# yhao-wang/DenseRetrievalToolkits

Hardware: AMD Instinct MI355X
Metric: queries/sec@top-1000, 10Mx768 corpus (BASELINE: passages encoded/sec + queries/sec@top-1000, 10Mx768 corpus, 1/2/4/8 GPU) (higher is better)
Workload: dtype bf16

## Files before the change

### denseretrievaltoolkits_amd/csrc/select.hip

```cpp
#include "profile.h"
#include "search_internal.h"

namespace drt {

constexpr int kSelThreads = 512;
constexpr int kSelWaves = kSelThreads / 64;
constexpr int kSelBins = 1024;
constexpr int kSelBuf = 4096;
constexpr int kSelKPT = 16;
constexpr int kSelRegCap = kSelKPT * kSelThreads;

template <int INPUT>
__device__ __forceinline__ uint64_t sel_load(const SelectArgs& a, int64_t q, int64_t j) {
  if (INPUT == SEL_KEYS64) return ((const uint64_t*)a.in)[q * a.in_stride + j];
  const uint32_t v = ((const uint32_t*)a.in)[q * a.in_stride + j];
  return ((uint64_t)v << 32) | (uint64_t)(uint32_t)j;
}

__device__ __forceinline__ float key_score(uint64_t x) { return desc_key_to_score((uint32_t)(x >> 32)); }

__device__ __forceinline__ int score_bin(float s, float smin, float scale) {
  if (scale == 0.0f) return 0;
  return hist_bin((s - smin) * scale, kSelBins, __builtin_signbit(s) ? 0 : kSelBins - 1);
}
// ... 41 lines not shown
#pragma unroll
  for (int size = 2; size <= N; size <<= 1) {
#pragma unroll
    for (int stride = size >> 1; stride > 0; stride >>= 1) {
      if (stride >= NT) {
        if (E >= 2 && stride == NT) sort_inthread<T, NT, E, 1>(v, size, tid);
        else if (E >= 4 && stride == 2 * NT) sort_inthread<T, NT, E, 2>(v, size, tid);
        else if (E >= 8) sort_inthread<T, NT, E, 4>(v, size, tid);
      } else {
        T p[E];
        if (stride >= 64) {
#pragma unroll
          for (int u = 0; u < E; ++u) buf[u * NT + tid] = v[u];
          __syncthreads();
#pragma unroll
          for (int u = 0; u < E; ++u) p[u] = buf[(u * NT + tid) ^ stride];
          __syncthreads();
        } else {
#pragma unroll
          for (int u = 0; u < E; ++u) p[u] = __shfl_xor(v[u], stride, 64);
        }
#pragma unroll
        for (int u = 0; u < E; ++u) {
          const int i = u * NT + tid;
          const bool keep_min = ((i & stride) == 0) == ((i & size) == 0);
          const T a = v[u], b = p[u];
          v[u] = keep_min ? (a < b ? a : b) : (a < b ? b : a);
        }
      }
    }
  }
#pragma unroll
  for (int u = 0; u < E; ++u) {
    const int i = u * NT + tid;
    if (i < n) buf[i] = v[u];
  }
  __syncthreads();
}

template <typename T, int NT>
__device__ __forceinline__ void block_sort(T* buf, int n) {
  if (n <= 1) {
    __syncthreads();
    return;
  }
  if (n <= NT) block_sort_fixed<T, NT, NT>(buf, n);
  else if (n <= 2 * NT) block_sort_fixed<T, NT, 2 * NT>(buf, n);
  else if (n <= 4 * NT) block_sort_fixed<T, NT, 4 * NT>(buf, n);
  else block_sort_fixed<T, NT, 8 * NT>(buf, n);
}

__device__ __forceinline__ void block_bitonic(uint64_t* buf, int n2) { block_sort<uint64_t, kSelThreads>(buf, n2); }

template <int INPUT, int OUTPUT>
__global__ __launch_bounds__(kSelThreads) void select_kernel(SelectArgs a) {
  __shared__ uint32_t hist[kSelWaves][kSelBins];
  __shared__ uint32_t suffix[kSelBins];
  __shared__ float fscr[kSelWaves];
  __shared__ uint64_t uscr[kSelWaves];
  __shared__ uint64_t sh_prefix, sh_mask;
  __shared__ int64_t sh_kk;
  __shared__ int sh_done, sh_bin;
  __shared__ uint32_t sh_nsel, sh_nside;
  __shared__ __attribute__((aligned(16))) uint64_t buf[kSelBuf];

  const int tid = threadIdx.x;
  const int wave = tid >> 6;
  const int64_t q = blockIdx.x;
  int64_t c_raw, c;
  if (INPUT == SEL_KEYS64) {
    c_raw = a.counts[q * kCntStride];
    c = c_raw < a.cap ? c_raw : a.cap;
  } else {
    c_raw = a.n_in;
    c = a.n_in;
  }
  const int64_t kk_total = (int64_t)a.k < c ? (int64_t)a.k : c;

  if (OUTPUT == SEL_KTH && (c < (int64_t)a.k || c == 0)) {
    if (tid == 0) a.tau[q] = -__builtin_inff();
    return;
  }

  bool fast_done = false;
  int nsel = 0;
  if (c > (int64_t)a.k && c <= kSelRegCap) {
    uint64_t kr[kSelKPT];
    float sc[kSelKPT];
#pragma unroll
    for (int u = 0; u < kSelKPT; ++u) {
      const int64_t j = (int64_t)u * kSelThreads + tid;
      const uint64_t x = sel_load<INPUT>(a, q, j < c ? j : 0);
      kr[u] = j < c ? x : ~0ull;
    }
    float lo = __builtin_inff(), hi = -__builtin_inff();
#pragma unroll
    for (int u = 0; u < kSelKPT; ++u) {
      sc[u] = key_score(kr[u]);
      if ((int64_t)u * kSelThreads + tid < c) {
        lo = fminf(lo, sc[u]);
        hi = fmaxf(hi, sc[u]);
      }
    }
    lo = block_reduce(lo, fscr, [](float x, float y) { return fminf(x, y); });
    hi = block_reduce(hi, fscr, [](float x, float y) { return fmaxf(x, y); });
    const float range = hi - lo;
    const float scale = hist_scale((float)kSelBins, range);
    for (int i = tid; i < kSelWaves * kSelBins; i += kSelThreads) (&hist[0][0])[i] = 0;
    __syncthreads();
    int bn[kSelKPT];
#pragma unroll
    for (int u = 0; u < kSelKPT; ++u) {
      bn[u] = -1;
      if ((int64_t)u * kSelThreads + tid < c) {
        bn[u] = score_bin(sc[u], lo, scale);
        atomicAdd(&hist[wave][bn[u]], 1u);
      }
    }
    __syncthreads();
    for (int i = tid; i < kSelBins; i += kSelThreads) {
      uint32_t t = 0;
#pragma unroll
      for (int w = 0; w < kSelWaves; ++w) t += hist[w][i];
      suffix[i] = t;
    }
    __syncthreads();
    for (int off = 1; off < kSelBins; off <<= 1) {
      uint32_t v[kSelBins / kSelThreads];
#pragma unroll
      for (int u = 0; u < kSelBins / kSelThreads; ++u) {
        const int i = tid + u * kSelThreads;
        v[u] = suffix[i] + (i + off < kSelBins ? suffix[i + off] : 0u);
      }
      __syncthreads();
#pragma unroll
      for (int u = 0; u < kSelBins / kSelThreads; ++u) suffix[tid + u * kSelThreads] = v[u];
      __syncthreads();
    }
    if (tid == 0) sh_bin = 0;
    __syncthreads();
    for (int i = tid; i < kSelBins; i += kSelThreads) {
      const bool ok = (int64_t)suffix[i] >= kk_total;
      const bool next_ok = (i + 1 < kSelBins) && (int64_t)suffix[i + 1] >= kk_total;
      if (ok && !next_ok) sh_bin = i;
    }
    __syncthreads();
    const int b = sh_bin;
    if (OUTPUT == SEL_KTH) {
      float t = __builtin_inff();
#pragma unroll
      for (int u = 0; u < kSelKPT; ++u)
        if (bn[u] >= b) t = fminf(t, sc[u]);
      t = block_reduce(t, fscr, [](float x, float y) { return fminf(x, y); });
      if (tid == 0) a.tau[q] = t;
      return;
    }
    const uint32_t cnt_sel = suffix[b];
    const uint32_t c_above = (b + 1 < kSelBins) ? suffix[b + 1] : 0u;
    const uint32_t cnt_b = cnt_sel - c_above;
    if (cnt_b <= (uint32_t)(kSelBuf / 2) && kk_total <= kSelBuf / 2) {
      uint64_t* side = buf + kSelBuf / 2;
      if (tid == 0) {
        sh_nsel = 0;
        sh_nside = 0;
      }
      __syncthreads();
#pragma unroll
      for (int u = 0; u < kSelKPT; ++u) {
        if (bn[u] > b) buf[atomicAdd(&sh_nsel, 1u)] = kr[u];
        else if (bn[u] == b) side[atomicAdd(&sh_nside, 1u)] = kr[u];
      }
      __syncthreads();
      const int ns = (int)sh_nside;
      int m2 = 1;
      while (m2 < ns) m2 <<= 1;
      for (int i = ns + tid; i < m2; i += kSelThreads) side[i] = ~0ull;
      __syncthreads();
      block_bitonic(side, m2);
      const int need = (int)kk_total - (int)c_above;
      for (int i = tid; i < need; i += kSelThreads) buf[c_above + i] = side[i];
      __syncthreads();
      nsel = (int)kk_total;
      fast_done = true;
    } else if (cnt_sel <= (uint32_t)kSelBuf) {
      if (tid == 0) sh_nsel = 0;
      __syncthreads();
#pragma unroll
      for (int u = 0; u < kSelKPT; ++u)
        if (bn[u] >= b) buf[atomicAdd(&sh_nsel, 1u)] = kr[u];
      __syncthreads();
      nsel = (int)sh_nsel;
      fast_done = true;
    }
  } else if (c > (int64_t)a.k) {
    float lo = __builtin_inff(), hi = -__builtin_inff();
    for (int64_t j = tid; j < c; j += kSelThreads) {
      const float s = key_score(sel_load<INPUT>(a, q, j));
      lo = fminf(lo, s);
      hi = fmaxf(hi, s);
    }
    lo = block_reduce(lo, fscr, [](float x, float y) { return fminf(x, y); });
    hi = block_reduce(hi, fscr, [](float x, float y) { return fmaxf(x, y); });
    const float range = hi - lo;
    const float scale = hist_scale((float)kSelBins, range);
    for (int i = tid; i < kSelWaves * kSelBins; i += kSelThreads) (&hist[0][0])[i] = 0;
    __syncthreads();
    for (int64_t j = tid; j < c; j += kSelThreads) {
      const float s = key_score(sel_load<INPUT>(a, q, j));
      atomicAdd(&hist[wave][score_bin(s, lo, scale)], 1u);
    }
    __syncthreads();
    for (int i = tid; i < kSelBins; i += kSelThreads) {
      uint32_t t = 0;
#pragma unroll
      for (int w = 0; w < kSelWaves; ++w) t += hist[w][i];
      suffix[i] = t;
    }
    __syncthreads();
    for (int off = 1; off < kSelBins; off <<= 1) {
      uint32_t v[kSelBins / kSelThreads];
#pragma unroll
      for (int u = 0; u < kSelBins / kSelThreads; ++u) {
        const int i = tid + u * kSelThreads;
        v[u] = suffix[i] + (i + off < kSelBins ? suffix[i + off] : 0u);
      }
      __syncthreads();
#pragma unroll
      for (int u = 0; u < kSelBins / kSelThreads; ++u) suffix[tid + u * kSelThreads] = v[u];
      __syncthreads();
    }
    if (tid == 0) sh_bin = 0;
    __syncthreads();
    for (int i = tid; i < kSelBins; i += kSelThreads) {
      const bool ok = (int64_t)suffix[i] >= kk_total;
      const bool next_ok = (i + 1 < kSelBins) && (int64_t)suffix[i + 1] >= kk_total;
      if (ok && !next_ok) sh_bin = i;
    }
    __syncthreads();
    const int b = sh_bin;
    const uint32_t cnt_sel = suffix[b];
    if (OUTPUT == SEL_KTH) {
      float t = __builtin_inff();
      for (int64_t j = tid; j < c; j += kSelThreads) {
        const float s = key_score(sel_load<INPUT>(a, q, j));
        if (score_bin(s, lo, scale) >= b) t = fminf(t, s);
      }
      t = block_reduce(t, fscr, [](float x, float y) { return fminf(x, y); });
      if (tid == 0) a.tau[q] = t;
      return;
    }
    const uint32_t c_above = (b + 1 < kSelBins) ? suffix[b + 1] : 0u;
    const uint32_t cnt_b = cnt_sel - c_above;
    if (cnt_b <= (uint32_t)(kSelBuf / 2) && kk_total <= kSelBuf / 2) {
      uint64_t* side = buf + kSelBuf / 2;
      if (tid == 0) {
        sh_nsel = 0;
        sh_nside = 0;
      }
      __syncthreads();
      for (int64_t j = tid; j < c; j += kSelThreads) {
        const uint64_t x = sel_load<INPUT>(a, q, j);
        const int bx = score_bin(key_score(x), lo, scale);
        if (bx > b) buf[atomicAdd(&sh_nsel, 1u)] = x;
        else if (bx == b) side[atomicAdd(&sh_nside, 1u)] = x;
      }
      __syncthreads();
      const int ns = (int)sh_nside;
      int m2 = 1;
      while (m2 < ns) m2 <<= 1;
      for (int i = ns + tid; i < m2; i += kSelThreads) side[i] = ~0ull;
      __syncthreads();
      block_bitonic(side, m2);
      const int need = (int)kk_total - (int)c_above;
      for (int i = tid; i < need; i += kSelThreads) buf[c_above + i] = side[i];
      __syncthreads();
      nsel = (int)kk_total;
      fast_done = true;
    } else if (cnt_sel <= (uint32_t)kSelBuf) {
      if (tid == 0) sh_nsel = 0;
      __syncthreads();
      for (int64_t j = tid; j < c; j += kSelThreads) {
        const uint64_t x = sel_load<INPUT>(a, q, j);
        if (score_bin(key_score(x), lo, scale) >= b) {
          const uint32_t p = atomicAdd(&sh_nsel, 1u);
          if (p < (uint32_t)kSelBuf) buf[p] = x;
        }
      }
      __syncthreads();
      nsel = (int)sh_nsel;
      fast_done = true;
    }
  }

  if (!fast_done) {
    if (tid == 0) {
      sh_prefix = 0;
      sh_mask = 0;
      sh_kk = kk_total;
      sh_done = (c <= (int64_t)a.k) ? 1 : 0;
      if (c <= (int64_t)a.k) {
        sh_prefix = ~0ull;
        sh_mask = ~0ull;
      }
    }
    __syncthreads();
    uint32_t* h0 = &hist[0][0];
    for (int shift = 56; shift >= 0 && !sh_done; shift -= 8) {
      for (int i = tid; i < 256; i += kSelThreads) h0[i] = 0;
      __syncthreads();
      const uint64_t prefix = sh_prefix, mask = sh_mask;
      for (int64_t j = tid; j < c; j += kSelThreads) {
        const uint64_t x = sel_load<INPUT>(a, q, j);
        if ((x & mask) == prefix) atomicAdd(&h0[(x >> shift) & 255], 1u);
      }
      __syncthreads();
      if (tid < 64) {
        const uint32_t b0 = h0[4 * tid], b1 = h0[4 * tid + 1], b2 = h0[4 * tid + 2], b3 = h0[4 * tid + 3];
        const uint32_t s4 = b0 + b1 + b2 + b3;
        uint32_t incl = s4;
#pragma unroll
        for (int o = 1; o < 64; o <<= 1) {
          const uint32_t v = __shfl_up(incl, o, 64);
          if (tid >= o) incl += v;
        }
        const uint32_t excl = incl - s4;
        const int64_t kk = sh_kk;
        if ((int64_t)excl < kk && kk <= (int64_t)incl) {
          uint32_t run = excl;
          const uint32_t bb[4] = {b0, b1, b2, b3};
          int d = 0;
          uint32_t cnt = 0;
#pragma unroll
          for (int t = 0; t < 4; ++t) {
            if ((int64_t)(run + bb[t]) >= kk) {
              d = 4 * tid + t;
              cnt = bb[t];
              break;
            }
            run += bb[t];
          }
          const int64_t rem = kk - run;
          sh_prefix = prefix | ((uint64_t)d << shift);
          sh_mask = mask | (255ull << shift);
          sh_kk = rem;
          if ((int64_t)cnt == rem) sh_done = 1;
        }
      }
      __syncthreads();
    }
    const uint64_t thr = sh_prefix | ~sh_mask;
    if (tid == 0) sh_nsel = 0;
    __syncthreads();
    for (int64_t j = tid; j < c; j += kSelThreads) {
      const uint64_t x = sel_load<INPUT>(a, q, j);
      if (x <= thr) {
        const uint32_t p = atomicAdd(&sh_nsel, 1u);
        if (p < (uint32_t)kSelBuf) buf[p] = x;
      }
    }
    __syncthreads();
    nsel = (int)sh_nsel;
  }

  nsel = nsel < kSelBuf ? nsel : kSelBuf;
  int n2 = 1;
  while (n2 < nsel) n2 <<= 1;
  for (int i = nsel + tid; i < n2; i += kSelThreads) buf[i] = ~0ull;
  __syncthreads();
  block_bitonic(buf, n2);

  const int64_t orow = a.qmap ? (int64_t)a.qmap[q] : q;
  if (a.out_packed) {
    uint64_t* op = a.out_packed + orow * (int64_t)(a.k + 1);
    for (int j = tid; j < a.k; j += kSelThreads) {
      if (j < kk_total) {
        const uint64_t x = buf[j];
        op[j] = (x & 0xFFFFFFFF00000000ull) | (uint64_t)(uint32_t)(a.id_offset + (int64_t)(x & 0xFFFFFFFFull));
      } else {
        op[j] = ~0ull;
      }
    }
    if (tid == 0) {
      const uint64_t nval = (uint64_t)(kk_total < a.k ? kk_total : a.k);
      bool bad = INPUT == SEL_KEYS64 && c_raw > a.cap;
      if (INPUT == SEL_KEYS64 && a.pass0) {
        const uint32_t* t = a.pass0 + q * 4;
        if (t[2] && (int64_t)t[1] + (c_raw - (int64_t)t[0]) < (int64_t)a.k) bad = true;
      }
      op[a.k] = (nval << 32) | (bad ? 1ull : 0ull) | (c_raw > (int64_t)a.k ? 2ull : 0ull);
    }
    return;
  }
  float* os = a.out_scores + orow * a.ldo;
  int64_t* oi = a.out_ids + orow * a.ldo;
  for (int j = tid; j < a.k; j += kSelThreads) {
    if (j < kk_total) {
      const uint64_t x = buf[j];
      os[j] = key_score(x);
      oi[j] = a.id_offset + (int64_t)(x & 0xFFFFFFFFull);
    } else {
      os[j] = kPadScore;
      oi[j] = -1;
    }
  }
  if (a.status && tid == 0) {
    int st = 0;
    if (INPUT == SEL_KEYS64) {
      if (c_raw > a.cap) st = 1;
      const int64_t kq = a.k_cert > 0 ? a.k_cert : a.k;
      if (!a.global_tau && c_raw < kq && c_raw < a.n_total) st = 1;
    }
    a.status[orow] = st;
  }
}

constexpr int kTightThreads = 256;

__global__ __launch_bounds__(kTightThreads) void tighten_kernel(const uint64_t* keys, int64_t cap,
                                                                const uint32_t* counts, const float* tau0, int r,
                                                                float* tau1, uint32_t* pass0) {
  __shared__ uint32_t hist[256];
  __shared__ uint32_t sh_prefix, sh_rem;
// ... 438 lines not shown
```

### denseretrievaltoolkits_amd/csrc/search.hip

```cpp
#include <cmath>

#include "profile.h"
#include "search_internal.h"

namespace drt {

constexpr int kHitCap = 1024;
constexpr int kTopRL = 4;

__host__ __device__ __forceinline__ int pass_tiles(int ntiles, int npass, int pass) {
  return npass <= 1 ? ntiles : (pass < ntiles ? (ntiles - 1 - pass) / npass + 1 : 0);
}

__device__ __forceinline__ void glds16(const void* gsrc, uint32_t lds_addr) {
  uint32_t keep;
  asm volatile(
      "s_mov_b32 %0, m0\n\t"
      "s_mov_b32 m0, %2\n\t"
      "s_nop 0\n\t"
      "global_load_lds_dwordx4 %1, off\n\t"
      "s_mov_b32 m0, %0"
      : "=&s"(keep)
      : "v"(gsrc), "s"(lds_addr)
      : "memory");
// ... 143 lines not shown
  }
  template <bool NT>
  __device__ __forceinline__ void issue(const ScanArgs& a, uint32_t slot_lds, const char* base, bool partial,
                                        int64_t tile, int wave, int lane) {
    if (partial) {
      issue_tile16<D, NW, NT>(a, slot_lds, tile, wave, lane);
      return;
    }
#define DRT_LEAN3(POL)                                                                                   \
  {                                                                                                     \
    uint32_t keep;                                                                                      \
    asm volatile(                                                                                       \
        "s_mov_b32 %0, m0\n\t"                                                                          \
        "s_mov_b32 m0, %2\n\t"                                                                          \
        "s_nop 0\n\t"                                                                                   \
        "global_load_lds_dwordx4 %3, %1" POL "\n\t"                                                     \
        "s_mov_b32 m0, %4\n\t"                                                                          \
        "s_nop 0\n\t"                                                                                   \
        "global_load_lds_dwordx4 %5, %1" POL "\n\t"                                                     \
        "s_mov_b32 m0, %6\n\t"                                                                          \
        "s_nop 0\n\t"                                                                                   \
        "global_load_lds_dwordx4 %7, %1" POL "\n\t"                                                     \
        "s_mov_b32 m0, %0"                                                                              \
        : "=&s"(keep)                                                                                   \
        : "s"(base), "s"(slot_lds + loff[0]), "v"(voff[0]), "s"(slot_lds + loff[1]), "v"(voff[1]),      \
          "s"(slot_lds + loff[2]), "v"(voff[2])                                                         \
        : "memory");                                                                                    \
  }
#define DRT_LEAN1(POL, J)                                                                                \
  {                                                                                                     \
    uint32_t keep;                                                                                      \
    asm volatile(                                                                                       \
        "s_mov_b32 %0, m0\n\t"                                                                          \
        "s_mov_b32 m0, %2\n\t"                                                                          \
        "s_nop 0\n\t"                                                                                   \
        "global_load_lds_dwordx4 %3, %1" POL "\n\t"                                                     \
        "s_mov_b32 m0, %0"                                                                              \
        : "=&s"(keep)                                                                                   \
        : "s"(base), "s"(slot_lds + loff[J]), "v"(voff[J])                                              \
        : "memory");                                                                                    \
  }
    if constexpr (G == 3) {
      if constexpr (NT) DRT_LEAN3(" nt")
      else DRT_LEAN3("")
    } else {
#pragma unroll
      for (int j = 0; j < G; ++j) {
        if constexpr (NT) DRT_LEAN1(" nt", j)
        else DRT_LEAN1("", j)
      }
    }
#undef DRT_LEAN3
#undef DRT_LEAN1
  }
};

template <int N>
__device__ __forceinline__ void wait_tiles_younger(int younger) {
  switch (younger) {
    case 0: asm volatile("s_waitcnt vmcnt(0)" ::: "memory"); break;
    case 1: asm volatile("s_waitcnt vmcnt(%0)" ::"n"(N) : "memory"); break;
    case 2: asm volatile("s_waitcnt vmcnt(%0)" ::"n"(2 * N) : "memory"); break;
    case 3: asm volatile("s_waitcnt vmcnt(%0)" ::"n"(3 * N < 63 ? 3 * N : 63) : "memory"); break;
    case 4: asm volatile("s_waitcnt vmcnt(%0)" ::"n"(4 * N < 63 ? 4 * N : 63) : "memory"); break;
    case 5: asm volatile("s_waitcnt vmcnt(%0)" ::"n"(5 * N < 63 ? 5 * N : 63) : "memory"); break;
    default: asm volatile("s_waitcnt vmcnt(%0)" ::"n"(6 * N < 63 ? 6 * N : 63) : "memory"); break;
  }
}

template <int D, int MODE, int NW = 8, bool AGG = true>
__global__ __launch_bounds__(NW * 64, 1) void ip_scan16_kernel(ScanArgs a) {
  using C = Scan16Cfg<D, NW>;
  constexpr int QB = 128 / (NW * 16);
  __shared__ __attribute__((aligned(16))) char smem[C::LDS_BYTES];
  uint64_t* hk = (uint64_t*)(smem + C::HIT_KEY_OFF);
  uint16_t* hq = (uint16_t*)(smem + C::HIT_Q_OFF);
  uint32_t* hit_n = (uint32_t*)(smem + C::HIT_N_OFF);
  uint32_t* qcnt = (uint32_t*)(smem + C::QCNT_OFF);
  uint32_t* qoff = qcnt + kQueriesPerWG;

  const int tid = threadIdx.x;
  const int wave = __builtin_amdgcn_readfirstlane(tid >> 6);
  const int lane = tid & 63;
  const int r = lane & 15;
  const int kq = lane >> 4;

  const int64_t qbase = (int64_t)blockIdx.y * kQueriesPerWG;
  const int64_t ntiles = (a.nrows + kT16 - 1) / kT16;
  const int64_t t0 = blockIdx.x;
  const int64_t tstep = gridDim.x;
  const int64_t my_tiles = t0 < ntiles ? (ntiles - 1 - t0) / tstep + 1 : 0;
  if (my_tiles == 0) return;
  if (MODE == SCAN_FILTER && tid == 0) *hit_n = 0;
  const uint32_t ring = lds_addr_of(smem);

  int qloc[QB];
  int64_t qg[QB];
  bool qok[QB];
  bf16x8 qf[C::KS][QB];
  float tau[QB];
#pragma unroll
  for (int b = 0; b < QB; ++b) {
    qloc[b] = wave * 16 * QB + 16 * b + r;
    qg[b] = qbase + qloc[b];
    qok[b] = qg[b] < a.nq;
    const int64_t qs = qok[b] ? qg[b] : 0;
// ... 364 lines not shown
  if (my_tiles & 1) epilogue(accA, rbA);
  else epilogue(accB, rbB);
  if (wcnt) wave_flush_hits(a, qw, hk, hq, wcnt, lane);
}

template <int D>
struct Scan32Cfg {
  static constexpr int KS = D / 32;
  static constexpr int RD = KS % 2 == 0 ? 2 : 1;
  static constexpr int TILE_BYTES = kT16 * D * 2;
  static constexpr int HIT_BYTES = kHitCap * 9;
  static constexpr int NB_RAW = (160 * 1024 - HIT_BYTES) / TILE_BYTES;
  static constexpr int NB = NB_RAW > 6 ? 6 : NB_RAW;
  static constexpr int RING_BYTES = NB * TILE_BYTES;
  static constexpr int LDS_BYTES = RING_BYTES + HIT_BYTES;
  static_assert(NB >= 3, "ring too small");
  static_assert(LDS_BYTES <= 160 * 1024, "LDS budget");
};
constexpr int kQueriesPerWG32 = 256;

template <int D>
__global__ __launch_bounds__(512, 1) void ip_scan32r_kernel(ScanArgs a) {
  constexpr int NW = 8;
  using C = Scan16Cfg<D, NW>;
  using C32 = Scan32Cfg<D>;
  constexpr int NB = C32::NB;
  constexpr int PD = NB - 2;
  static_assert(NB == 6, "the pair protocol's slot census");
  constexpr int KS = C32::KS;
  constexpr int RD = C32::RD;
  constexpr int kSeg = kHitCap / NW;
  __shared__ __attribute__((aligned(16))) char smem[C32::LDS_BYTES];

  const int tid = threadIdx.x;
  const int wave = __builtin_amdgcn_readfirstlane(tid >> 6);
  const int lane = tid & 63;
  const int r = lane & 15;
  const int kq = lane >> 4;
  uint64_t* hk = (uint64_t*)(smem + C32::RING_BYTES) + wave * kSeg;
  uint8_t* hq = (uint8_t*)(smem + C32::RING_BYTES + kHitCap * 8) + wave * kSeg;

  const int64_t qbase = (int64_t)blockIdx.y * kQueriesPerWG32;
  const int tmul = a.npass > 1 ? a.npass : 1;
  const int tph = a.npass > 1 ? a.pass : 0;
  const int tall = (int)((a.nrows + kT16 - 1) / kT16);
  const int ntiles = pass_tiles(tall, a.npass, a.pass);
  const uint32_t nrows = (uint32_t)a.nrows;
  const int t0 = blockIdx.x;
  const int tstep = gridDim.x;
  const int my_tiles = t0 < ntiles ? (ntiles - 1 - t0) / tstep + 1 : 0;
  if (my_tiles == 0) return;
  const int partial_tile = ((a.nrows & (kT16 - 1)) != 0 && (tall - 1) % tmul == tph) ? ntiles - 1 : -1;
  const uint32_t ring = lds_addr_of(smem);
  const int64_t tile_stride = (int64_t)tstep * tmul * kT16 * a.ldp * 2;
  const char* next_base = (const char*)(a.P + ((int64_t)t0 * tmul + tph) * kT16 * a.ldp);

  const int64_t qw = qbase + wave * 32;
  bf16x8 qf0[KS], qf1[KS];
  float tau0, tau1;
  {
    const int64_t g0 = qw + r, g1 = qw + 16 + r;
    const bool ok0 = g0 < a.nq, ok1 = g1 < a.nq;
    const int64_t s0 = ok0 ? g0 : 0, s1 = ok1 ? g1 : 0;
#pragma unroll
    for (int s = 0; s < KS; ++s) {
      qf0[s] = *(const bf16x8*)(a.Q + s0 * a.ldq + s * 32 + kq * 8);
      qf1[s] = *(const bf16x8*)(a.Q + s1 * a.ldq + s * 32 + kq * 8);
    }
    const float v0 = a.tau[s0], v1 = a.tau[s1];
    tau0 = ok0 ? v0 : __builtin_nanf("");
    tau1 = ok1 ? v1 : __builtin_nanf("");
    if (!ok0) {
#pragma unroll
      for (int s = 0; s < KS; ++s) qf0[s] = (bf16x8){};
    }
    if (!ok1) {
#pragma unroll
      for (int s = 0; s < KS; ++s) qf1[s] = (bf16x8){};
    }
  }
#pragma unroll
  for (int s = 0; s < KS; ++s) asm volatile("" ::"v"(qf0[s]), "v"(qf1[s]));
  asm volatile("" ::"v"(tau0), "v"(tau1));
  asm volatile("s_waitcnt vmcnt(0)" ::: "memory");

  LeanTile<D, NW> lt;
  lt.init(a, wave, lane);
#pragma unroll
  for (int p = 0; p < PD; ++p) {
    if (p < my_tiles) {
      const int tile = t0 + p * tstep;
      lt.template issue<false>(a, ring + p * C::TILE_BYTES, next_base, tile == partial_tile, tile * tmul + tph, wave,
                               lane);
      next_base += tile_stride;
    }
  }
  if (wave >= NW / 2) __builtin_amdgcn_s_setprio(1);
  if (PD <= my_tiles) wait_vmcnt<C::GLDS_PER_WAVE>();
  else wait_vmcnt<0>();
  lds_barrier();

  const int sw = (r >> 1) & 7;
  int aoff[2];
#pragma unroll
  for (int m = 0; m < 2; ++m) aoff[m] = r * 128 + (((4 * m + kq) ^ sw) << 4);
  auto frag = [&](int slot, int s) -> bf16x8 {
    return *(const bf16x8*)(smem + slot * C::TILE_BYTES + (s >> 1) * (kT16 * 128) + aoff[s & 1]);
  };
  bf16x8 af[RD];
#pragma unroll
  for (int s = 0; s < RD; ++s) af[s] = frag(0, s);

  int wcnt = 0;
  auto append = [&](const f32x4& acc, float tau, int ql, uint32_t rowbase) {
    const float mx = fmaxf(fmaxf(acc[0], acc[1]), fmaxf(acc[2], acc[3])) - tau;
    if (__ballot(mx >= 0.0f) == 0ull) return;
#pragma unroll
    for (int j = 0; j < 4; ++j) {
      const bool hit = acc[j] >= tau && rowbase + j < nrows;
      const uint64_t m = __ballot(hit);
      if (m == 0ull) continue;
      const int c = __builtin_popcountll(m);
      if (wcnt + c > kSeg) {
        wave_flush_hits(a, qw, hk, hq, wcnt, lane);
        wcnt = 0;
      }
      if (hit) {
        const int pos = wcnt + (int)__builtin_amdgcn_mbcnt_hi((uint32_t)(m >> 32),
                                                              __builtin_amdgcn_mbcnt_lo((uint32_t)m, 0u));
        hk[pos] = ((uint64_t)desc_key(acc[j]) << 32) | (uint64_t)(a.row_base + rowbase + j);
        hq[pos] = (uint8_t)ql;
      }
      wcnt += c;
    }
  };

  auto epilogue = [&](const f32x4& p0, const f32x4& p1, uint32_t rowbase) {
    append(p0, tau0, r, rowbase);
    append(p1, tau1, 16 + r, rowbase);
  };

  int buf = 0;
  auto pair_sync = [&](int it) {
    if (it + PD <= my_tiles) wait_vmcnt<C::GLDS_PER_WAVE>();
    else wait_vmcnt<0>();
    lds_barrier();
  };
  auto iter = [&](int it, f32x4& acc0, f32x4& acc1, uint32_t& rb, const f32x4& prev0, const f32x4& prev1,
                  uint32_t rb_prev) {
    const int tile = t0 + it * tstep;
    const bool do_dma = it + PD < my_tiles;
    const int ntile = tile + PD * tstep;
    const int pslot = buf < 2 ? buf + NB - 2 : buf - 2;
    const int nslot = buf + 1 == NB ? 0 : buf + 1;
    acc0 = (f32x4){0.f, 0.f, 0.f, 0.f};
    acc1 = (f32x4){0.f, 0.f, 0.f, 0.f};
#pragma unroll
    for (int s = 0; s < KS; ++s) {
      acc0 = __builtin_amdgcn_mfma_f32_16x16x32_bf16(af[s % RD], qf0[s], acc0, 0, 0, 0);
      acc1 = __builtin_amdgcn_mfma_f32_16x16x32_bf16(af[s % RD], qf1[s], acc1, 0, 0, 0);
      af[s % RD] = s + RD < KS ? frag(buf, s + RD) : frag(nslot, s + RD - KS);
      __builtin_amdgcn_sched_barrier(0);
      if (s == KS / 4 && do_dma) {
        lt.template issue<false>(a, ring + pslot * C::TILE_BYTES, next_base, ntile == partial_tile,
                                 ntile * tmul + tph, wave, lane);
        next_base += tile_stride;
      }
      __builtin_amdgcn_sched_barrier(0);
    }
    if (it > 0) epilogue(prev0, prev1, rb_prev);
    rb = (uint32_t)(tile * tmul + tph) * kT16 + 4 * kq;
    buf = nslot;
  };
  f32x4 a0, a1, b0, b1;
  uint32_t rbA = 0, rbB = 0;
  for (int it = 0; it < my_tiles; it += 2) {
    if (it > 0) pair_sync(it);
    iter(it, a0, a1, rbA, b0, b1, rbB);
    if (it + 1 < my_tiles) iter(it + 1, b0, b1, rbB, a0, a1, rbA);
  }
  if (my_tiles & 1) epilogue(a0, a1, rbA);
  else epilogue(b0, b1, rbB);
  if (wcnt) wave_flush_hits(a, qw, hk, hq, wcnt, lane);
}

struct TopkPlan : PlanHead {
  int64_t n, k, nq, nq_pad;
  bool sample;
  int64_t cap;
  int64_t m;
  int64_t stride;
  int64_t r;
  int64_t nchunk;
  int64_t kc;
  size_t off_cs, off_ci, off_delta, off_rcnt, total;
};

static size_t plan_refine_tail(TopkPlan& p) {
  p.kc = refine_width(p.k);
  WsBump b{p.head_end};
  p.off_cs = b.take((size_t)p.nq_pad * p.kc * 4);
  p.off_ci = b.take((size_t)p.nq_pad * p.kc * 8);
  p.off_delta = b.take((size_t)p.nq_pad * p.kc * 4);
  p.off_rcnt = b.take((size_t)p.nq_pad * 8);
  return b.o;
}

static double poisson_tail_ge(double lam, int64_t r) {
  double logp = -lam + r * std::log(lam) - std::lgamma((double)r + 1.0);
  double p = std::exp(logp), s = 0.0;
  for (int64_t i = r; i < r + 2000; ++i) {
    s += p;
    p *= lam / (double)(i + 1);
    if (p < 1e-30 * s) break;
  }
  return s;
}


static TopkPlan make_plan(int64_t nq, int64_t n, int64_t k) {
// ... 665 lines not shown
```

Before: 86480.

## Restructure top-k select: aliased LDS, wave-ballot appends, rank-based placement skipping final sort

Rewrites the per-query select kernel. The per-wave histogram now aliases the shared output buffer, which cuts LDS use. Per-element shared atomics become wave-aggregated ballot appends, and the log-step suffix scan becomes a shuffle-based scan. The register path is templated on items per thread (4/8/16) to match the candidate count. When bins above the threshold are small, elements are placed by counting-rank into bin-ordered runs and the small boundary bin is rank-sorted, so the final bitonic sort can be skipped. This adds code complexity and special cases, and rank loops with O(n) per element could cost more when bins are dense.

```diff
diff --git a/denseretrievaltoolkits_amd/csrc/select.hip b/denseretrievaltoolkits_amd/csrc/select.hip
--- a/denseretrievaltoolkits_amd/csrc/select.hip
+++ b/denseretrievaltoolkits_amd/csrc/select.hip
@@ -117,17 +117,241 @@
 
 __device__ __forceinline__ void block_bitonic(uint64_t* buf, int n2) { block_sort<uint64_t, kSelThreads>(buf, n2); }
 
+typedef uint32_t __attribute__((may_alias)) sel_u32;
+typedef u32x4 __attribute__((may_alias)) sel_u32x4;
+
+struct SelLds {
+  sel_u32* hist;
+  uint32_t* suffix;
+  uint32_t* fill;
+  int* big;
+  float* flo;
+  float* fhi;
+  uint32_t* wsum;
+  int* bin;
+  uint32_t* nsel;
+  uint32_t* nside;
+  uint64_t* buf;
+};
+
+__device__ __forceinline__ void sel_range_and_clear(float& lo, float& hi, const SelLds& L) {
+  const int tid = threadIdx.x;
+#pragma unroll
+  for (int o = 32; o > 0; o >>= 1) lo = fminf(lo, __shfl_xor(lo, o, 64));
+#pragma unroll
+  for (int o = 32; o > 0; o >>= 1) hi = fmaxf(hi, __shfl_xor(hi, o, 64));
+  if ((tid & 63) == 0) {
+    L.flo[tid >> 6] = lo;
+    L.fhi[tid >> 6] = hi;
+  }
+  if (tid == 0) {
+    *L.bin = 0;
+    *L.nsel = 0;
+    *L.nside = 0;
+    *L.big = 0;
+  }
+  for (int i = tid; i < kSelBins; i += kSelThreads) L.fill[i] = 0;
+  sel_u32x4* h4 = (sel_u32x4*)L.hist;
+  const u32x4 z = {0u, 0u, 0u, 0u};
+  for (int i = tid; i < kSelWaves * kSelBins / 4; i += kSelThreads) h4[i] = z;
+  __syncthreads();
+  lo = L.flo[0];
+  hi = L.fhi[0];
+#pragma unroll
+  for (int i = 1; i < kSelWaves; ++i) {
+    lo = fminf(lo, L.flo[i]);
+    hi = fmaxf(hi, L.fhi[i]);
+  }
+}
+
+__device__ __forceinline__ int sel_suffix_bin(const SelLds& L, int64_t kk_total) {
+  const int tid = threadIdx.x, lane = tid & 63, wave = tid >> 6;
+  uint32_t t0 = 0, t1 = 0;
+#pragma unroll
+  for (int w = 0; w < kSelWaves; ++w) {
+    t0 += L.hist[w * kSelBins + 2 * tid];
+    t1 += L.hist[w * kSelBins + 2 * tid + 1];
+  }
+  const uint32_t pair = t0 + t1;
+  uint32_t s = pair;
+#pragma unroll
+  for (int o = 1; o < 64; o <<= 1) {
+    const uint32_t v = __shfl_down(s, o, 64);
+    if (lane + o < 64) s += v;
+  }
+  if (lane == 0) L.wsum[wave] = s;
+  __syncthreads();
+#pragma unroll
+  for (int w = 1; w < kSelWaves; ++w)
+    if (w > wave) s += L.wsum[w];
+  const uint32_t s1 = s - t0, s2 = s - pair;
+  L.suffix[2 * tid] = s;
+  L.suffix[2 * tid + 1] = s1;
+  const bool ok0 = (int64_t)s >= kk_total, ok1 = (int64_t)s1 >= kk_total;
+  const bool ok2 = 2 * tid + 2 < kSelBins && (int64_t)s2 >= kk_total;
+  if (ok1 && !ok2) *L.bin = 2 * tid + 1;
+  else if (ok0 && !ok1) *L.bin = 2 * tid;
+  __syncthreads();
+  return *L.bin;
+}
+
+__device__ __forceinline__ uint32_t lanes_below(uint64_t m) {
+  return __builtin_amdgcn_mbcnt_hi((uint32_t)(m >> 32), __builtin_amdgcn_mbcnt_lo((uint32_t)m, 0u));
+}
+
+__device__ __forceinline__ uint32_t wave_append_slot(bool pred, uint32_t* counter) {
+  const uint64_t m = __ballot(pred);
+  uint32_t base = 0;
+  if ((threadIdx.x & 63) == 0 && m != 0) base = atomicAdd(counter, (uint32_t)__popcll(m));
+  return (uint32_t)__builtin_amdgcn_readfirstlane((int)base) + lanes_below(m);
+}
+
+constexpr int kSelSideRank = 128;
+constexpr int kSelBinRank = 128;
+
+__device__ __forceinline__ void sel_take_side(uint64_t* side, int ns, int need, uint64_t* dst) {
+  const int tid = threadIdx.x;
+  if (ns <= kSelSideRank) {
+    if (tid < ns) {
+      const uint64_t x = side[tid];
+      int r = 0;
+      for (int i = 0; i < ns; ++i) r += side[i] < x ? 1 : 0;
+      if (r < need) dst[r] = x;
+    }
+    __syncthreads();
+    return;
+  }
+  int m2 = 1;
+  while (m2 < ns) m2 <<= 1;
+  for (int i = ns + tid; i < m2; i += kSelThreads) side[i] = ~0ull;
+  __syncthreads();
+  block_bitonic(side, m2);
+  for (int i = tid; i < need; i += kSelThreads) dst[i] = side[i];
+  __syncthreads();
+}
+
+template <int INPUT, int OUTPUT, int KPT>
+__device__ __forceinline__ int select_in_registers(const SelectArgs& a, int64_t q, int64_t c, int64_t kk_total,
+                                                   const SelLds& L, float* fscr, int& nsel) {
+  const int tid = threadIdx.x, wave = tid >> 6, lane = tid & 63;
+  uint64_t kr[KPT];
+  float sc[KPT];
+#pragma unroll
+  for (int u = 0; u < KPT; ++u) {
+    const int64_t j = (int64_t)u * kSelThreads + tid;
+    const uint64_t x = sel_load<INPUT>(a, q, j < c ? j : 0);
+    kr[u] = j < c ? x : ~0ull;
+  }
+  float lo = __builtin_inff(), hi = -__builtin_inff();
+#pragma unroll
+  for (int u = 0; u < KPT; ++u) {
+    sc[u] = key_score(kr[u]);
+    if ((int64_t)u * kSelThreads + tid < c) {
+      lo = fminf(lo, sc[u]);
+      hi = fmaxf(hi, sc[u]);
+    }
+  }
+  sel_range_and_clear(lo, hi, L);
+  const float range = hi - lo;
+  const float scale = hist_scale((float)kSelBins, range);
+  int bn[KPT];
+#pragma unroll
+  for (int u = 0; u < KPT; ++u) {
+    bn[u] = -1;
+    if ((int64_t)u * kSelThreads + tid < c) {
+      bn[u] = score_bin(sc[u], lo, scale);
+      atomicAdd(&L.hist[wave * kSelBins + bn[u]], 1u);
+    }
+  }
+  __syncthreads();
+  const int b = sel_suffix_bin(L, kk_total);
+  if (OUTPUT == SEL_KTH) {
+    float t = __builtin_inff();
+#pragma unroll
+    for (int u = 0; u < KPT; ++u)
+      if (bn[u] >= b) t = fminf(t, sc[u]);
+    t = block_reduce(t, fscr, [](float x, float y) { return fminf(x, y); });
+    if (tid == 0) a.tau[q] = t;
+    return 2;
+  }
+  const uint32_t cnt_sel = L.suffix[b];
+  const uint32_t c_above = (b + 1 < kSelBins) ? L.suffix[b + 1] : 0u;
+  const uint32_t cnt_b = cnt_sel - c_above;
+  const bool split = cnt_b <= (uint32_t)(kSelBuf / 2) && kk_total <= kSelBuf / 2;
+  if (!split && cnt_sel > (uint32_t)kSelBuf) return 0;
+  if (!split) {
+    uint32_t nh = 0;
+#pragma unroll
+    for (int u = 0; u < KPT; ++u) nh += (uint32_t)__popcll(__ballot(bn[u] >= b));
+    uint32_t oh = 0;
+    if (lane == 0 && nh) oh = atomicAdd(L.nsel, nh);
+    oh = (uint32_t)__builtin_amdgcn_readfirstlane((int)oh);
+#pragma unroll
+    for (int u = 0; u < KPT; ++u) {
+      const uint64_t mh = __ballot(bn[u] >= b);
+      if (bn[u] >= b) L.buf[oh + lanes_below(mh)] = kr[u];
+      oh += (uint32_t)__popcll(mh);
+    }
+    __syncthreads();
+    nsel = (int)cnt_sel;
+    return 1;
+  }
+  const bool apart = cnt_sel <= (uint32_t)(kSelBuf / 2) && cnt_b <= (uint32_t)kSelSideRank;
+  uint64_t* runs = apart ? L.buf + kSelBuf / 2 : L.buf;
+  uint64_t* side = apart ? runs + c_above : L.buf + kSelBuf / 2;
+  uint32_t nb = 0;
+#pragma unroll
+  for (int u = 0; u < KPT; ++u) nb += (uint32_t)__popcll(__ballot(bn[u] == b));
+  uint32_t ob = 0;
+  if (lane == 0 && nb) ob = atomicAdd(L.nside, nb);
+  ob = (uint32_t)__builtin_amdgcn_readfirstlane((int)ob);
+#pragma unroll
+  for (int u = 0; u < KPT; ++u) {
+    const uint64_t mb = __ballot(bn[u] == b);
+    if (bn[u] > b) {
+      const uint32_t st = bn[u] + 1 < kSelBins ? L.suffix[bn[u] + 1] : 0u;
+      if (L.suffix[bn[u]] - st > (uint32_t)kSelBinRank) *L.big = 1;
+      runs[st + atomicAdd(&L.fill[bn[u]], 1u)] = kr[u];
+    } else if (bn[u] == b) {
+      side[ob + lanes_below(mb)] = kr[u];
+    }
+    ob += (uint32_t)__popcll(mb);
+  }
+  __syncthreads();
+  nsel = (int)kk_total;
+  const bool ranked = apart && *L.big == 0;
+  if (ranked) {
+#pragma unroll
+    for (int u = 0; u < KPT; ++u) {
+      if (bn[u] > b) {
+        const uint32_t st = bn[u] + 1 < kSelBins ? L.suffix[bn[u] + 1] : 0u;
+        const uint32_t n = L.suffix[bn[u]] - st;
+        uint32_t r = 0;
+#pragma nounroll
+        for (uint32_t i = 0; i < n; ++i) r += runs[st + i] < kr[u] ? 1u : 0u;
+        L.buf[st + r] = kr[u];
+      }
+    }
+  } else if (apart) {
+    for (int i = tid; i < (int)c_above; i += kSelThreads) L.buf[i] = runs[i];
+  }
+  sel_take_side(side, (int)cnt_b, (int)kk_total - (int)c_above, L.buf + c_above);
+  return ranked ? 3 : 1;
+}
+
 template <int INPUT, int OUTPUT>
 __global__ __launch_bounds__(kSelThreads) void select_kernel(SelectArgs a) {
-  __shared__ uint32_t hist[kSelWaves][kSelBins];
+  __shared__ __attribute__((aligned(16))) uint64_t buf[kSelBuf];
   __shared__ uint32_t suffix[kSelBins];
-  __shared__ float fscr[kSelWaves];
-  __shared__ uint64_t uscr[kSelWaves];
+  __shared__ float fscr[kSelWaves], flo[kSelWaves], fhi[kSelWaves];
+  __shared__ uint32_t wsum[kSelWaves];
   __shared__ uint64_t sh_prefix, sh_mask;
   __shared__ int64_t sh_kk;
   __shared__ int sh_done, sh_bin;
   __shared__ uint32_t sh_nsel, sh_nside;
-  __shared__ __attribute__((aligned(16))) uint64_t buf[kSelBuf];
+  __shared__ uint32_t fill[kSelBins];
+  __shared__ int sh_big;
+  const SelLds L = {(sel_u32*)buf, suffix, fill, &sh_big, flo, fhi, wsum, &sh_bin, &sh_nsel, &sh_nside, buf};
 
   const int tid = threadIdx.x;
   const int wave = tid >> 6;
@@ -148,115 +372,16 @@
   }
 
   bool fast_done = false;
+  bool sorted = false;
   int nsel = 0;
   if (c > (int64_t)a.k && c <= kSelRegCap) {
-    uint64_t kr[kSelKPT];
-    float sc[kSelKPT];
-#pragma unroll
-    for (int u = 0; u < kSelKPT; ++u) {
-      const int64_t j = (int64_t)u * kSelThreads + tid;
-      const uint64_t x = sel_load<INPUT>(a, q, j < c ? j : 0);
-      kr[u] = j < c ? x : ~0ull;
-    }
-    float lo = __builtin_inff(), hi = -__builtin_inff();
-#pragma unroll
-    for (int u = 0; u < kSelKPT; ++u) {
-      sc[u] = key_score(kr[u]);
-      if ((int64_t)u * kSelThreads + tid < c) {
-        lo = fminf(lo, sc[u]);
-        hi = fmaxf(hi, sc[u]);
-      }
-    }
-    lo = block_reduce(lo, fscr, [](float x, float y) { return fminf(x, y); });
-    hi = block_reduce(hi, fscr, [](float x, float y) { return fmaxf(x, y); });
-    const float range = hi - lo;
-    const float scale = hist_scale((float)kSelBins, range);
-    for (int i = tid; i < kSelWaves * kSelBins; i += kSelThreads) (&hist[0][0])[i] = 0;
-    __syncthreads();
-    int bn[kSelKPT];
-#pragma unroll
-    for (int u = 0; u < kSelKPT; ++u) {
-      bn[u] = -1;
-      if ((int64_t)u * kSelThreads + tid < c) {
-        bn[u] = score_bin(sc[u], lo, scale);
-        atomicAdd(&hist[wave][bn[u]], 1u);
-      }
-    }
-    __syncthreads();
-    for (int i = tid; i < kSelBins; i += kSelThreads) {
-      uint32_t t = 0;
-#pragma unroll
-      for (int w = 0; w < kSelWaves; ++w) t += hist[w][i];
-      suffix[i] = t;
-    }
-    __syncthreads();
-    for (int off = 1; off < kSelBins; off <<= 1) {
-      uint32_t v[kSelBins / kSelThreads];
-#pragma unroll
-      for (int u = 0; u < kSelBins / kSelThreads; ++u) {
-        const int i = tid + u * kSelThreads;
-        v[u] = suffix[i] + (i + off < kSelBins ? suffix[i + off] : 0u);
-      }
-      __syncthreads();
-#pragma unroll
-      for (int u = 0; u < kSelBins / kSelThreads; ++u) suffix[tid + u * kSelThreads] = v[u];
-      __syncthreads();
-    }
-    if (tid == 0) sh_bin = 0;
-    __syncthreads();
-    for (int i = tid; i < kSelBins; i += kSelThreads) {
-      const bool ok = (int64_t)suffix[i] >= kk_total;
-      const bool next_ok = (i + 1 < kSelBins) && (int64_t)suffix[i + 1] >= kk_total;
-      if (ok && !next_ok) sh_bin = i;
-    }
-    __syncthreads();
-    const int b = sh_bin;
-    if (OUTPUT == SEL_KTH) {
-      float t = __builtin_inff();
-#pragma unroll
-      for (int u = 0; u < kSelKPT; ++u)
-        if (bn[u] >= b) t = fminf(t, sc[u]);
-      t = block_reduce(t, fscr, [](float x, float y) { return fminf(x, y); });
-      if (tid == 0) a.tau[q] = t;
-      return;
-    }
-    const uint32_t cnt_sel = suffix[b];
-    const uint32_t c_above = (b + 1 < kSelBins) ? suffix[b + 1] : 0u;
-    const uint32_t cnt_b = cnt_sel - c_above;
-    if (cnt_b <= (uint32_t)(kSelBuf / 2) && kk_total <= kSelBuf / 2) {
-      uint64_t* side = buf + kSelBuf / 2;
-      if (tid == 0) {
-        sh_nsel = 0;
-        sh_nside = 0;
-      }
-      __syncthreads();
-#pragma unroll
-      for (int u = 0; u < kSelKPT; ++u) {
-        if (bn[u] > b) buf[atomicAdd(&sh_nsel, 1u)] = kr[u];
-        else if (bn[u] == b) side[atomicAdd(&sh_nside, 1u)] = kr[u];
-      }
-      __syncthreads();
-      const int ns = (int)sh_nside;
-      int m2 = 1;
-      while (m2 < ns) m2 <<= 1;
-      for (int i = ns + tid; i < m2; i += kSelThreads) side[i] = ~0ull;
-      __syncthreads();
-      block_bitonic(side, m2);
-      const int need = (int)kk_total - (int)c_above;
-      for (int i = tid; i < need; i += kSelThreads) buf[c_above + i] = side[i];
-      __syncthreads();
-      nsel = (int)kk_total;
-      fast_done = true;
-    } else if (cnt_sel <= (uint32_t)kSelBuf) {
-      if (tid == 0) sh_nsel = 0;
-      __syncthreads();
-#pragma unroll
-      for (int u = 0; u < kSelKPT; ++u)
-        if (bn[u] >= b) buf[atomicAdd(&sh_nsel, 1u)] = kr[u];
-      __syncthreads();
-      nsel = (int)sh_nsel;
-      fast_done = true;
-    }
+    int r;
+    if (c <= 4 * kSelThreads) r = select_in_registers<INPUT, OUTPUT, 4>(a, q, c, kk_total, L, fscr, nsel);
+    else if (c <= 8 * kSelThreads) r = select_in_registers<INPUT, OUTPUT, 8>(a, q, c, kk_total, L, fscr, nsel);
+    else r = select_in_registers<INPUT, OUTPUT, kSelKPT>(a, q, c, kk_total, L, fscr, nsel);
+    if (r == 2) return;
+    fast_done = r != 0;
+    sorted = r == 3;
   } else if (c > (int64_t)a.k) {
     float lo = __builtin_inff(), hi = -__builtin_inff();
     for (int64_t j = tid; j < c; j += kSelThreads) {
@@ -264,45 +389,15 @@
       lo = fminf(lo, s);
       hi = fmaxf(hi, s);
     }
-    lo = block_reduce(lo, fscr, [](float x, float y) { return fminf(x, y); });
-    hi = block_reduce(hi, fscr, [](float x, float y) { return fmaxf(x, y); });
+    sel_range_and_clear(lo, hi, L);
     const float range = hi - lo;
     const float scale = hist_scale((float)kSelBins, range);
-    for (int i = tid; i < kSelWaves * kSelBins; i += kSelThreads) (&hist[0][0])[i] = 0;
-    __syncthreads();
     for (int64_t j = tid; j < c; j += kSelThreads) {
       const float s = key_score(sel_load<INPUT>(a, q, j));
-      atomicAdd(&hist[wave][score_bin(s, lo, scale)], 1u);
-    }
-    __syncthreads();
-    for (int i = tid; i < kSelBins; i += kSelThreads) {
-      uint32_t t = 0;
-#pragma unroll
-      for (int w = 0; w < kSelWaves; ++w) t += hist[w][i];
-      suffix[i] = t;
-    }
-    __syncthreads();
-    for (int off = 1; off < kSelBins; off <<= 1) {
-      uint32_t v[kSelBins / kSelThreads];
-#pragma unroll
-      for (int u = 0; u < kSelBins / kSelThreads; ++u) {
-        const int i = tid + u * kSelThreads;
-        v[u] = suffix[i] + (i + off < kSelBins ? suffix[i + off] : 0u);
-      }
-      __syncthreads();
-#pragma unroll
-      for (int u = 0; u < kSelBins / kSelThreads; ++u) suffix[tid + u * kSelThreads] = v[u];
-      __syncthreads();
-    }
-    if (tid == 0) sh_bin = 0;
-    __syncthreads();
-    for (int i = tid; i < kSelBins; i += kSelThreads) {
-      const bool ok = (int64_t)suffix[i] >= kk_total;
-      const bool next_ok = (i + 1 < kSelBins) && (int64_t)suffix[i + 1] >= kk_total;
-      if (ok && !next_ok) sh_bin = i;
-    }
-    __syncthreads();
-    const int b = sh_bin;
+      atomicAdd(&L.hist[wave * kSelBins + score_bin(s, lo, scale)], 1u);
+    }
+    __syncthreads();
+    const int b = sel_suffix_bin(L, kk_total);
     const uint32_t cnt_sel = suffix[b];
     if (OUTPUT == SEL_KTH) {
       float t = __builtin_inff();
@@ -316,43 +411,27 @@
     }
     const uint32_t c_above = (b + 1 < kSelBins) ? suffix[b + 1] : 0u;
     const uint32_t cnt_b = cnt_sel - c_above;
-    if (cnt_b <= (uint32_t)(kSelBuf / 2) && kk_total <= kSelBuf / 2) {
+    const bool split = cnt_b <= (uint32_t)(kSelBuf / 2) && kk_total <= kSelBuf / 2;
+    if (split || cnt_sel <= (uint32_t)kSelBuf) {
       uint64_t* side = buf + kSelBuf / 2;
-      if (tid == 0) {
-        sh_nsel = 0;
-        sh_nside = 0;
+      for (int64_t j0 = 0; j0 < c; j0 += kSelThreads) {
+        const int64_t j = j0 + tid;
+        const uint64_t x = sel_load<INPUT>(a, q, j < c ? j : 0);
+        const int bx = j < c ? score_bin(key_score(x), lo, scale) : -1;
+        const bool ph = split ? bx > b : bx >= b;
+        const bool pb = split && bx == b;
+        const uint32_t sh = wave_append_slot(ph, &sh_nsel);
+        const uint32_t sb = wave_append_slot(pb, &sh_nside);
+        if (ph && sh < (uint32_t)kSelBuf) buf[sh] = x;
+        if (pb) side[sb] = x;
       }
       __syncthreads();
-      for (int64_t j = tid; j < c; j += kSelThreads) {
-        const uint64_t x = sel_load<INPUT>(a, q, j);
-        const int bx = score_bin(key_score(x), lo, scale);
-        if (bx > b) buf[atomicAdd(&sh_nsel, 1u)] = x;
-        else if (bx == b) side[atomicAdd(&sh_nside, 1u)] = x;
-      }
-      __syncthreads();
-      const int ns = (int)sh_nside;
-      int m2 = 1;
-      while (m2 < ns) m2 <<= 1;
-      for (int i = ns + tid; i < m2; i += kSelThreads) side[i] = ~0ull;
-      __syncthreads();
-      block_bitonic(side, m2);
-      const int need = (int)kk_total - (int)c_above;
-      for (int i = tid; i < need; i += kSelThreads) buf[c_above + i] = side[i];
-      __syncthreads();
-      nsel = (int)kk_total;
-      fast_done = true;
-    } else if (cnt_sel <= (uint32_t)kSelBuf) {
-      if (tid == 0) sh_nsel = 0;
-      __syncthreads();
-      for (int64_t j = tid; j < c; j += kSelThreads) {
-        const uint64_t x = sel_load<INPUT>(a, q, j);
-        if (score_bin(key_score(x), lo, scale) >= b) {
-          const uint32_t p = atomicAdd(&sh_nsel, 1u);
-          if (p < (uint32_t)kSelBuf) buf[p] = x;
-        }
-      }
-      __syncthreads();
-      nsel = (int)sh_nsel;
+      if (split) {
+        sel_take_side(side, (int)cnt_b, (int)kk_total - (int)c_above, buf + c_above);
+        nsel = (int)kk_total;
+      } else {
+        nsel = (int)sh_nsel;
+      }
       fast_done = true;
     }
   }
@@ -369,7 +448,7 @@
       }
     }
     __syncthreads();
-    uint32_t* h0 = &hist[0][0];
+    sel_u32* h0 = L.hist;
     for (int shift = 56; shift >= 0 && !sh_done; shift -= 8) {
       for (int i = tid; i < 256; i += kSelThreads) h0[i] = 0;
       __syncthreads();
@@ -416,23 +495,25 @@
     const uint64_t thr = sh_prefix | ~sh_mask;
     if (tid == 0) sh_nsel = 0;
     __syncthreads();
-    for (int64_t j = tid; j < c; j += kSelThreads) {
-      const uint64_t x = sel_load<INPUT>(a, q, j);
-      if (x <= thr) {
-        const uint32_t p = atomicAdd(&sh_nsel, 1u);
-        if (p < (uint32_t)kSelBuf) buf[p] = x;
-      }
+    for (int64_t j0 = 0; j0 < c; j0 += kSelThreads) {
+      const int64_t j = j0 + tid;
+      const uint64_t x = sel_load<INPUT>(a, q, j < c ? j : 0);
+      const bool take = j < c && x <= thr;
+      const uint32_t p = wave_append_slot(take, &sh_nsel);
+      if (take && p < (uint32_t)kSelBuf) buf[p] = x;
     }
     __syncthreads();
     nsel = (int)sh_nsel;
   }
 
-  nsel = nsel < kSelBuf ? nsel : kSelBuf;
-  int n2 = 1;
-  while (n2 < nsel) n2 <<= 1;
-  for (int i = nsel + tid; i < n2; i += kSelThreads) buf[i] = ~0ull;
-  __syncthreads();
-  block_bitonic(buf, n2);
+  if (!sorted) {
+    nsel = nsel < kSelBuf ? nsel : kSelBuf;
+    int n2 = 1;
+    while (n2 < nsel) n2 <<= 1;
+    for (int i = nsel + tid; i < n2; i += kSelThreads) buf[i] = ~0ull;
+    __syncthreads();
+    block_bitonic(buf, n2);
+  }
 
   const int64_t orow = a.qmap ? (int64_t)a.qmap[q] : q;
   if (a.out_packed) {
```

Result: no change. 86910, median of 6 (+0.5%).

## Restrict tile DMA issue to half the waves in the scan kernel

Applied to the files above, without the earlier changes.

Introduces a HalfTile loader in which only the upper half of the waves (the ones already given raised priority) issue the global-to-LDS loads for each corpus tile, each handling more pieces through one inline-asm block with m0 offsets. The other waves only compute and wait with vmcnt(0). The DMA issue point moves earlier in the K loop. The aim is to take load-issue overhead off half the waves and cut per-wave VMEM instruction pressure, at the cost of uneven load distribution and a changed wait pattern.

```diff
diff --git a/denseretrievaltoolkits_amd/csrc/search.hip b/denseretrievaltoolkits_amd/csrc/search.hip
--- a/denseretrievaltoolkits_amd/csrc/search.hip
+++ b/denseretrievaltoolkits_amd/csrc/search.hip
@@ -219,6 +219,58 @@
     }
 #undef DRT_LEAN3
 #undef DRT_LEAN1
+  }
+};
+
+template <int D>
+struct HalfTile {
+  using C = Scan16Cfg<D, 4>;
+  static constexpr bool kOk = C::GLDS_PER_TILE % 4 == 0 && C::GLDS_PER_TILE <= 24;
+  static constexpr int G = C::GLDS_PER_TILE / 4;
+  uint32_t voff;
+  uint32_t loff;
+  __device__ __forceinline__ void init(const ScanArgs& a, int wave, int lane) {
+    const int lw = wave & 3;
+    const int row = ((lw & 1) << 3) + (lane >> 3);
+    const int c = (lane & 7) ^ ((row >> 1) & 7);
+    voff = (uint32_t)((row * a.ldp + (lw >> 1) * 64 + c * 8) * 2);
+    loff = (uint32_t)__builtin_amdgcn_readfirstlane(lw * 1024);
+  }
+  __device__ __forceinline__ void issue(const ScanArgs& a, uint32_t slot_lds, const char* base, bool partial,
+                                        int tile, int wave, int lane) {
+    static_assert(kOk, "loader half: a multiple of four pieces per tile");
+    uint32_t v = voff;
+    if (partial) {
+      const int row = ((wave & 1) << 3) + (lane >> 3);
+      const int last = (int)(a.nrows - 1 - (int64_t)tile * kT16);
+      if (row > last) v -= (uint32_t)((row - last) * a.ldp * 2);
+    }
+    const uint32_t l0 = slot_lds + loff;
+    uint32_t keep;
+#define DRT_HALF_PIECE(LDS, OFF) \
+  "s_add_u32 m0, %2, " #LDS "\n\ts_nop 0\n\tglobal_load_lds_dwordx4 %3, %1 offset:" #OFF "\n\t"
+#define DRT_HALF_ISSUE(PIECES) \
+  asm volatile("s_mov_b32 %0, m0\n\t" PIECES "s_mov_b32 m0, %0" : "=&s"(keep) : "s"(base), "s"(l0), "v"(v) : "memory", "scc")
+#define DRT_HP0 DRT_HALF_PIECE(0, 0)
+#define DRT_HP1 DRT_HP0 DRT_HALF_PIECE(3840, 256)
+#define DRT_HP2 DRT_HP1 DRT_HALF_PIECE(7680, 512)
+#define DRT_HP3 DRT_HP2 DRT_HALF_PIECE(11520, 768)
+#define DRT_HP4 DRT_HP3 DRT_HALF_PIECE(15360, 1024)
+#define DRT_HP5 DRT_HP4 DRT_HALF_PIECE(19200, 1280)
+    if constexpr (G == 1) DRT_HALF_ISSUE(DRT_HP0);
+    else if constexpr (G == 2) DRT_HALF_ISSUE(DRT_HP1);
+    else if constexpr (G == 3) DRT_HALF_ISSUE(DRT_HP2);
+    else if constexpr (G == 4) DRT_HALF_ISSUE(DRT_HP3);
+    else if constexpr (G == 5) DRT_HALF_ISSUE(DRT_HP4);
+    else DRT_HALF_ISSUE(DRT_HP5);
+#undef DRT_HP5
+#undef DRT_HP4
+#undef DRT_HP3
+#undef DRT_HP2
+#undef DRT_HP1
+#undef DRT_HP0
+#undef DRT_HALF_ISSUE
+#undef DRT_HALF_PIECE
   }
 };
 
@@ -689,6 +741,10 @@
   if (my_tiles == 0) return;
   const int partial_tile = ((a.nrows & (kT16 - 1)) != 0 && (tall - 1) % tmul == tph) ? ntiles - 1 : -1;
   const uint32_t ring = lds_addr_of(smem);
+  constexpr bool HALVES = HalfTile<D>::kOk;
+  constexpr int GW = HALVES ? HalfTile<D>::G : C::GLDS_PER_WAVE;
+  constexpr int KDMA = HALVES ? KS / 12 : KS / 4;
+  const bool loader = !HALVES || wave >= NW / 2;
   const int64_t tile_stride = (int64_t)tstep * tmul * kT16 * a.ldp * 2;
   const char* next_base = (const char*)(a.P + ((int64_t)t0 * tmul + tph) * kT16 * a.ldp);
 
@@ -722,19 +778,27 @@
   asm volatile("s_waitcnt vmcnt(0)" ::: "memory");
 
   LeanTile<D, NW> lt;
-  lt.init(a, wave, lane);
+  HalfTile<D> ht;
+  if constexpr (HALVES) ht.init(a, wave, lane);
+  else lt.init(a, wave, lane);
+  auto issue = [&](int slot, int tile) {
+    if constexpr (HALVES)
+      ht.issue(a, ring + slot * C::TILE_BYTES, next_base, tile == partial_tile, tile * tmul + tph, wave, lane);
+    else
+      lt.template issue<false>(a, ring + slot * C::TILE_BYTES, next_base, tile == partial_tile, tile * tmul + tph,
+                               wave, lane);
+    next_base += tile_stride;
+  };
+  auto pair_wait = [&](int it) {
+    if (loader && it + PD <= my_tiles) wait_vmcnt<GW>();
+    else wait_vmcnt<0>();
+  };
 #pragma unroll
   for (int p = 0; p < PD; ++p) {
-    if (p < my_tiles) {
-      const int tile = t0 + p * tstep;
-      lt.template issue<false>(a, ring + p * C::TILE_BYTES, next_base, tile == partial_tile, tile * tmul + tph, wave,
-                               lane);
-      next_base += tile_stride;
-    }
+    if (p < my_tiles && loader) issue(p, t0 + p * tstep);
   }
   if (wave >= NW / 2) __builtin_amdgcn_s_setprio(1);
-  if (PD <= my_tiles) wait_vmcnt<C::GLDS_PER_WAVE>();
-  else wait_vmcnt<0>();
+  pair_wait(0);
   lds_barrier();
 
   const int sw = (r >> 1) & 7;
@@ -779,14 +843,13 @@
 
   int buf = 0;
   auto pair_sync = [&](int it) {
-    if (it + PD <= my_tiles) wait_vmcnt<C::GLDS_PER_WAVE>();
-    else wait_vmcnt<0>();
+    pair_wait(it);
     lds_barrier();
   };
   auto iter = [&](int it, f32x4& acc0, f32x4& acc1, uint32_t& rb, const f32x4& prev0, const f32x4& prev1,
                   uint32_t rb_prev) {
     const int tile = t0 + it * tstep;
-    const bool do_dma = it + PD < my_tiles;
+    const bool do_dma = it + PD < my_tiles && loader;
     const int ntile = tile + PD * tstep;
     const int pslot = buf < 2 ? buf + NB - 2 : buf - 2;
     const int nslot = buf + 1 == NB ? 0 : buf + 1;
@@ -798,11 +861,7 @@
       acc1 = __builtin_amdgcn_mfma_f32_16x16x32_bf16(af[s % RD], qf1[s], acc1, 0, 0, 0);
       af[s % RD] = s + RD < KS ? frag(buf, s + RD) : frag(nslot, s + RD - KS);
       __builtin_amdgcn_sched_barrier(0);
-      if (s == KS / 4 && do_dma) {
-        lt.template issue<false>(a, ring + pslot * C::TILE_BYTES, next_base, ntile == partial_tile,
-                                 ntile * tmul + tph, wave, lane);
-        next_base += tile_stride;
-      }
+      if (s == KDMA && do_dma) issue(pslot, ntile);
       __builtin_amdgcn_sched_barrier(0);
     }
     if (it > 0) epilogue(prev0, prev1, rb_prev);
```

Result: faster. 83770 before, 85450 after (median of 6 runs) (+2.0%).
